# shiyao-li/NextBestPath

Hardware: AMD Instinct MI355X
Metric: exploration steps/s (+ NBP maps/s) at 256x256 (higher is better)
Workload: dtype f32

## Files before the change

include/nbp_hip.h:

```cpp
#ifndef NBP_HIP_H
#define NBP_HIP_H

#include <stddef.h>
#include <stdint.h>

#ifdef __cplusplus
extern "C" {
#endif

#define NBP_E_ARG      (-1)
#define NBP_E_WS       (-2)
#define NBP_E_SHAPE    (-3)

int nbp_abi_version(void);
int nbp_device_info(char* arch_host, int arch_len, int* cu_count_host);
int nbp_tuning_active(void);
int nbp_tuning_report(char* buf_host, int len);
int nbp_tile_kernel_symbol(int tile, char* buf_host, int len);

#define NBP_N_CONV 48

typedef struct nbp_weights nbp_weights;

size_t nbp_packed_weights_bytes(void);
// ... 57 lines not shown
int nbp_conv3x3_split_f32(const float* src0, int C0, const float* src1, int C1, int ups, int B, int H, int W,
                          const void* w_planes, const void* wamax, int N, const float* scale, const float* shift, int relu,
                          float* out, const void* amax_in_or_null, void* amax_out_or_null, int split_k, void* ws,
                          size_t ws_bytes, void* stream);
size_t nbp_conv_first_wgrad_workspace_bytes(void);
int nbp_conv_first_wgrad_f32(const float* x_nchw, int B, int H, int W, const float* dy, float* dw, void* ws, size_t ws_bytes, void* stream);
int nbp_prepack_weights_split(const void* descs_dev, int n, void* wamax_words, void* stream);
int nbp_prepack_desc_bytes(void);
int nbp_pack_conv_weight_split_prezeroed(const float* w_oihw, int N, int C, int ksize, int c_total, void* dst_planes,
                                         void* wamax_zeroed, void* stream);
int nbp_pack_conv_weight_split_dgrad_known(const float* w_oihw, int N, int C, int c_total, void* dst_planes, const void* wamax_known,
                                           void* stream);
int nbp_pack_upconv_weight_split_dgrad(const float* w_oihw, int N, int C, void* dst_planes, void* wamax_out, void* stream);
size_t nbp_upconv_split_dgrad_workspace_bytes(int B, int H, int W, int N, int C);
int nbp_upconv3x3_split_dgrad_f32(const float* dy, int N, int B, int H, int W, const void* planes, const void* wamax, int C,
                                  const float* scale, const float* shift, float* dx, const void* amax_in, void* amax_out_or_null,
                                  void* ws, size_t ws_bytes, void* stream);
size_t nbp_upconv_wgrad_split_workspace_bytes(int B, int Hs, int Ws, int C, int N);
int nbp_upconv_wgrad_split_f32(const float* x, int C, int B, int Hs, int Ws, const float* dy, int N, float* dw,
                               const void* amax_x, const void* amax_y, void* ws, size_t ws_bytes, void* stream);
int nbp_conv1x1_split_f32(const float* src, int C, long long M, const void* w_planes, const void* wamax, int N,
                          const float* scale, const float* shift, int relu, float* out, const void* amax_in, void* stream);
int nbp_pack_conv1x1_weight_split_dgrad(const float* w_nc, int N, int C, void* dst_planes, void* wamax_out, void* stream);
int nbp_pack_conv_weight_split_dgrad(const float* w_oihw, int N, int C, int c_total, void* dst_planes, void* wamax_out, void* stream);

int nbp_conv_bn_part_rows(int B, int H, int W);
int nbp_conv3x3_split_bn_f32(const float* src0, int C0, const float* src1, int C1, int ups, int B, int H, int W,
                             const void* w_planes, const void* wamax, int N, const float* scale, const float* shift, int relu,
                             float* out, const void* amax_in_or_null, void* amax_out_or_null, int split_k, void* ws,
                             size_t ws_bytes, double* bn_part, int* bn_rows, void* stream);
int nbp_upconv3x3_split_bn_f32(const float* src, int C, int B, int H, int W, const void* planes_up, const void* wamax_up, int N,
                               const float* scale, const float* shift, int relu, float* out, const void* amax_in_or_null,
                               void* amax_out_or_null, int split_k, void* ws, size_t ws_bytes, double* bn_part, int* bn_rows,
                               void* stream);
int nbp_pack_conv_weight_split_h1(const float* w_oihw, int N, int C, int ksize, const float* scale_or_null, int c_off,
                                  int c_total, void* dst_planes, void* wamax_out, void* stream);
int nbp_pack_conv_weight_split_prezeroed_h1(const float* w_oihw, int N, int C, int ksize, int c_total, void* dst_planes,
                                            void* wamax_zeroed, void* stream);
int nbp_pack_conv_weight_split_dgrad_h1(const float* w_oihw, int N, int C, int c_total, void* dst_planes, void* wamax_out, void* stream);
int nbp_pack_conv_weight_split_dgrad_known_h1(const float* w_oihw, int N, int C, int c_total, void* dst_planes, const void* wamax_known,
                                              void* stream);
int nbp_pack_upconv_weight_split_h1(const float* w_oihw, int N, int C, void* dst_planes, void* wamax_out, void* stream);
int nbp_pack_upconv_weight_split_dgrad_h1(const float* w_oihw, int N, int C, void* dst_planes, void* wamax_out, void* stream);
int nbp_pack_conv1x1_weight_split_dgrad_h1(const float* w_nc, int N, int C, void* dst_planes, void* wamax_out, void* stream);
int nbp_prepack_weights_split_h1(const void* descs_dev, int n, void* wamax_words, void* stream);
int nbp_conv3x3_split_f32_h1(const float* src0, int C0, const float* src1, int C1, int ups, int B, int H, int W,
// ... 362 lines not shown
```

nextbestpath_amd/_lib.py:

```python
from __future__ import annotations

import ctypes as C
import os
import threading

HERE = os.path.dirname(os.path.abspath(__file__))
LIB_PATH = os.path.join(HERE, "libnbp_hip.so")

_vp, _i, _ll, _f, _sz, _d = C.c_void_p, C.c_int, C.c_longlong, C.c_float, C.c_size_t, C.c_double

SIGNATURES = {
    "nbp_abi_version": (_i, []),
    "nbp_device_info": (_i, [C.c_char_p, _i, C.POINTER(_i)]),
    "nbp_tuning_active": (_i, []),
    "nbp_tuning_report": (_i, [C.c_char_p, _i]),
    "nbp_tile_kernel_symbol": (_i, [_i, C.c_char_p, _i]),
    "nbp_packed_weights_bytes": (_sz, []),
    "nbp_pack_weights": (_i, [C.POINTER(_vp), C.POINTER(_vp), C.POINTER(_vp), _vp, _sz, _vp, C.POINTER(_vp)]),
    "nbp_free_weights": (None, [_vp]),
    "nbp_forward_workspace_bytes": (_sz, [_i, _i]),
    "nbp_forward_f32": (_i, [_vp, _vp, _i, _i, _vp, _vp, _vp, _sz, _vp]),
    "nbp_forward_flops": (_d, [_i, _i]),
    "nbp_conv_igemm_f32": (_i, [_vp, _i, _vp, _i, _i, _i, _i, _i, _i, _vp, _i, _vp, _vp, _i, _vp, _i, _i, _vp,
                                _sz, _vp]),
# ... 97 lines not shown
SIGNATURES["nbp_amax_f32"] = (_i, [_vp, _ll, _vp, _vp])
SIGNATURES["nbp_pack_upconv_weight_split"] = (_i, [_vp, _i, _i, _vp, _vp, _vp])
SIGNATURES["nbp_upconv3x3_split_f32"] = (_i, [_vp, _i, _i, _i, _i, _vp, _vp, _i, _vp, _vp, _i, _vp, _vp, _vp, _i, _vp, _sz, _vp])
SIGNATURES["nbp_conv_split_workspace_bytes"] = SIGNATURES["nbp_conv_igemm_workspace_bytes"]
SIGNATURES["nbp_conv_split_planned_workspace_bytes"] = (_sz, [_i, _i, _i, _i, _i, _i, _vp])
SIGNATURES["nbp_conv_split_planned_workspace_bytes_k"] = (_sz, [_i, _i, _i, _i, _i, _i, _i, _vp])
SIGNATURES["nbp_conv3x3_split_f32"] = (_i, [_vp, _i, _vp, _i, _i, _i, _i, _i, _vp, _vp, _i, _vp, _vp, _i, _vp, _vp, _vp, _i, _vp,
                                            _sz, _vp])
SIGNATURES["nbp_pack_upconv_weight_split_dgrad"] = (_i, [_vp, _i, _i, _vp, _vp, _vp])
SIGNATURES["nbp_upconv_split_dgrad_workspace_bytes"] = (_sz, [_i, _i, _i, _i, _i])
SIGNATURES["nbp_upconv3x3_split_dgrad_f32"] = (_i, [_vp, _i, _i, _i, _i, _vp, _vp, _i, _vp, _vp, _vp, _vp, _vp, _vp, _sz, _vp])
SIGNATURES["nbp_upconv_wgrad_split_workspace_bytes"] = (_sz, [_i, _i, _i, _i, _i])
SIGNATURES["nbp_upconv_wgrad_split_f32"] = (_i, [_vp, _i, _i, _i, _i, _vp, _i, _vp, _vp, _vp, _vp, _sz, _vp])
SIGNATURES["nbp_pack_conv_weight_split_prezeroed"] = (_i, [_vp, _i, _i, _i, _i, _vp, _vp, _vp])
SIGNATURES["nbp_pack_conv_weight_split_dgrad_known"] = (_i, [_vp, _i, _i, _i, _vp, _vp, _vp])
SIGNATURES["nbp_prepack_weights_split"] = (_i, [_vp, _i, _vp, _vp])
SIGNATURES["nbp_prepack_desc_bytes"] = (_i, [])
SIGNATURES["nbp_rowscale_amax_f32"] = (_i, [_vp, _vp, _ll, _i, _vp, _vp, _vp])
SIGNATURES["nbp_conv_first_linear_f32"] = (_i, [_vp, _i, _i, _i, _vp, _vp, _vp, _vp, _vp])
SIGNATURES["nbp_conv_first_wgrad_workspace_bytes"] = (_sz, [])
SIGNATURES["nbp_conv_first_wgrad_f32"] = (_i, [_vp, _i, _i, _i, _vp, _vp, _vp, _sz, _vp])
SIGNATURES["nbp_conv1x1_split_f32"] = (_i, [_vp, _i, _ll, _vp, _vp, _i, _vp, _vp, _i, _vp, _vp, _vp])
SIGNATURES["nbp_pack_conv1x1_weight_split_dgrad"] = (_i, [_vp, _i, _i, _vp, _vp, _vp])
SIGNATURES["nbp_pack_conv_weight_split_dgrad"] = (_i, [_vp, _i, _i, _i, _vp, _vp, _vp])
SIGNATURES["nbp_conv_bn_part_rows"] = (_i, [_i, _i, _i])
SIGNATURES["nbp_conv3x3_split_bn_f32"] = (_i, [_vp, _i, _vp, _i, _i, _i, _i, _i, _vp, _vp, _i, _vp, _vp, _i, _vp, _vp, _vp, _i, _vp,
                                               _sz, _vp, C.POINTER(_i), _vp])
SIGNATURES["nbp_upconv3x3_split_bn_f32"] = (_i, [_vp, _i, _i, _i, _i, _vp, _vp, _i, _vp, _vp, _i, _vp, _vp, _vp, _i, _vp, _sz, _vp,
                                                 C.POINTER(_i), _vp])
SIGNATURES["nbp_bn_train_forward_part4_f32"] = (_i, [_vp, _ll, _i, _vp, _vp, _f, _f, _vp, _vp, _i, _vp, _vp, _vp, _vp, _vp, _i, _vp, _i, _vp, _vp])
for _n in ("nbp_pack_conv_weight_split", "nbp_pack_conv_weight_split_prezeroed", "nbp_pack_conv_weight_split_dgrad",
           "nbp_pack_conv_weight_split_dgrad_known", "nbp_pack_upconv_weight_split", "nbp_pack_upconv_weight_split_dgrad",
           "nbp_pack_conv1x1_weight_split_dgrad", "nbp_prepack_weights_split", "nbp_conv3x3_split_f32", "nbp_conv3x3_split_bn_f32",
           "nbp_upconv3x3_split_f32", "nbp_upconv3x3_split_bn_f32", "nbp_upconv3x3_split_dgrad_f32", "nbp_conv1x1_split_f32",
           "nbp_upconv_wgrad_split_f32", "nbp_conv_wgrad_split_f32"):
    SIGNATURES[_n + "_h1"] = SIGNATURES[_n]
SIGNATURES["nbp_conv_igemm_bf16"] = SIGNATURES["nbp_conv_igemm_f32"]
SIGNATURES["nbp_conv_igemm_bf16_workspace_bytes"] = SIGNATURES["nbp_conv_igemm_workspace_bytes"]
SIGNATURES["nbp_pack_conv_weight_bf16"] = SIGNATURES["nbp_pack_conv_weight"]
SIGNATURES["nbp_f32_to_bf16"] = (_i, [_vp, _ll, _vp, _vp])
SIGNATURES["nbp_bf16_to_f32"] = (_i, [_vp, _ll, _vp, _vp])
_fpp, _ipp = C.POINTER(_f), C.POINTER(_i)
SIGNATURES["nbp_scene_fill_workspace_bytes"] = (_sz, [_fpp, _ipp, _i, _ll, _d])
SIGNATURES["nbp_scene_fill_cells_f32"] = (_i, [_vp, _ll, _vp, _fpp, _ipp, _i, _d, _i, C.c_uint, _vp, _vp, _vp, _sz, _vp])
SIGNATURES["nbp_scene_gather_f32"] = (_i, [_vp, _vp, _i, _i, _vp, _ll, _vp, _vp])
SIGNATURES["nbp_scene_coverage_workspace_bytes"] = (_sz, [_fpp, _ipp, _i, _d])
# ... 82 lines not shown
            fn.argtypes = args
        _lib = handle
    return _lib


_ERR = {-1: "NBP_E_ARG (bad argument)", -2: "NBP_E_WS (workspace too small)", -3: "NBP_E_SHAPE (unsupported shape)"}


def check(rc: int, what: str) -> None:
    if rc != 0:
        msg = _ERR.get(rc, f"hipError_t {rc}" if rc > 0 else f"error {rc}")
        raise NbpHipError(f"{what} failed: {msg}")


def ptr(t) -> int:
    if t is None:
        return 0
    if not t.is_contiguous():
        raise ValueError("tensor passed to the HIP path must be contiguous")
    return t.data_ptr()


_knobs = {}
NUMERICS_KNOBS = {"NBP_CONV_PRECISION", "NBP_SPLIT_MAX_K", "NBP_SPLIT_MAX_K_SMALL", "NBP_GATE_PSI", "NBP_CONV_HEAD", "NBP_BF16_PSI",
                  "NBP_BF16_FUSE"}


def tuning_active() -> bool:
    return os.environ.get("NBP_TUNING") == "1"


def tune(name: str, default: str) -> str:
    v = default
    if tuning_active():
        e = os.environ.get(name)
        if e is not None and e != "":
            v = e
    _knobs[name] = (default, v)
    return v


def effective_knobs() -> dict:
    out = {k: v for k, (d, v) in _knobs.items() if v != d}
    if _lib is not None:
        buf = C.create_string_buffer(4096)
        if _lib.nbp_tuning_report(buf, 4096) > 0:
            for item in buf.value.decode().split(","):
# ... 18 lines not shown
```

nextbestpath_amd/csrc/nbp_forward.hip:

```cpp
#include "common.h"
#include "nbp_internal.h"
#include <stdio.h>
#include <stdlib.h>
#include <string.h>

namespace {

enum Kind { K_FIRST, K_CONV3, K_ATT_G, K_ATT_X, K_PSI, K_FINAL };
struct LayerSpec { Kind kind; int cin, cout, k; };

struct Table {
    LayerSpec L[NBP_N_CONV];
    size_t w_off[NBP_N_CONV];
    size_t s_off[NBP_N_CONV], t_off[NBP_N_CONV];
    size_t total_floats;
    size_t w3_off[NBP_N_CONV];
    size_t w3u_off[NBP_N_CONV];
    bool is_up[NBP_N_CONV];
    int up_rank[NBP_N_CONV];
    size_t total3_bytes;
    size_t wup16_off[NBP_N_CONV], total_up16_bytes;
    size_t w1_off[NBP_N_CONV];
    int gate_rank[NBP_N_CONV];
    Table() {
// ... 377 lines not shown
                    int H, int ks, int N, void* ws, size_t wsb, hipStream_t st) {
        if (ks == 1 && C1 == C0 && C0 % 64 == 0 && !ups && h->w1[li[0]] && (!o2 || h->w1[li[1]])) {
            const long long M = (long long)B * H * H;
            ConvOperandsSplit s[2];
            for (int g = 0; g < (o2 ? 2 : 1); ++g) {
                const Ops& q = g ? *o2 : o;
                s[g] = ConvOperandsSplit{q.src0, q.src1, h->w1[li[g]], q.scale, q.shift, q.out, nullptr, nullptr, h->wamax1[li[g]], nullptr,
                                         nullptr, nullptr};
                int rc = ctx.ensure(q.src0, M * C0, &s[g].amax0);
                if (!rc) rc = ctx.ensure(q.src1, M * C1, &s[g].amax1);
                if (rc) return rc;
            }
            GatePsi psi;
            for (int g = 0; g < 2; ++g) {
                const int l = li[(g && o2) ? 1 : 0] + 2;
                psi.wpsi[g] = (const float*)h->w[l]; psi.st[g] = h->scale[l]; psi.gated[g] = ctx.gated[(g && o2) ? 1 : 0];
            }
            unsigned* gslot[2] = {nullptr, nullptr};
            if (ctx.gated[0]) for (int g = 0; g < (o2 ? 2 : 1); ++g) psi.gated_amax[g] = gslot[g] = ctx.unbound();
            static const int psi_on_load = nbp_tune_int("NBP_SPLIT_PSI_ON_LOAD", 1);
            const ConvPlan pc = nbp_plan_conv_split(M, C0, (C0 + C0) / 32 * 9, 0, o2 ? 2 : 1, H, H, 3, 0);
            psi.psi_only = psi_on_load && (C0 >= 128 || psi_on_load >= 2) && ctx.gated[0] && gslot[0] && (!o2 || gslot[1]) && pc.tile != 0 &&
                           M * C0 * 4 < (1ll << 31);
            int fused = 0;
            const int rc = nbp_gate1x1_split_launch_g(s[0], o2 ? &s[1] : nullptr, C0, M, N, 1, st, ctx.gated[0] ? &psi : nullptr, &fused);
            if (fused) {
                ctx.gated_taken = true;
                for (int g = 0; g < (o2 ? 2 : 1); ++g) {
                    if (gslot[g]) ctx.bind(ctx.gated[g], gslot[g]);
                    else ctx.alias(ctx.gated[g], (g ? *o2 : o).src1);
                    if (psi.psi_only) { ctx.psi_key[g] = ctx.gated[g]; ctx.psi_x[g] = (g ? *o2 : o).src1; }
                }
            }
            return rc;
        }
        const ConvPlan p = nbp_plan_conv_split((long long)B * H * H, N, (C0 + C1) / 32 * ks * ks, 0, o2 ? 2 : 1, H, H, ks, ups);
        if (!p.tile) return PathF32::conv(ctx, h, li, o, o2, C0, C1, ups, B, H, ks, N, ws, wsb, st);
        const long long hw = (long long)B * (ups ? H / 2 : H) * (ups ? H / 2 : H);
        ConvOperandsSplit s[2];
        for (int g = 0; g < (o2 ? 2 : 1); ++g) {
            const Ops& q = g ? *o2 : o;
            s[g] = ConvOperandsSplit{q.src0, q.src1, h->w3[li[g]], q.scale, q.shift, q.out, nullptr, nullptr, h->wamax[li[g]], nullptr,
                                     h->w3u[li[g]], h->wamax_u[li[g]]};
            int rc = ctx.ensure(q.src0, hw * C0, &s[g].amax0);
            if (!rc && C1) rc = ctx.ensure(q.src1, hw * C1, &s[g].amax1);
            if (rc) return rc;
// ... 339 lines not shown
```

nextbestpath_amd/csrc/nbp_internal.h:

```cpp
#pragma once
#include "common.h"

typedef unsigned short bf16_t;

enum { NBP_TILE_AUTO = 0, NBP_TILE_128x128 = 1, NBP_TILE_256x64 = 2, NBP_TILE_256x32 = 3, NBP_TILE_128x64 = 4,
       NBP_TILE_64x128 = 5,
       NBP_TILE_HALO_128 = 6, NBP_TILE_HALO_64 = 7,
       NBP_TILE_HALO4_128 = 8, NBP_TILE_HALO4_64 = 9,
       NBP_TILE_SPLIT_HALO_64 = 10, NBP_TILE_SPLIT_UP = 11,
       NBP_TILE_HALO_UP_128 = 12, NBP_TILE_HALO_UP_64 = 13,
       NBP_TILE_RESERVED_14 = 14,
       NBP_TILE_SPLIT_HALO_R8 = 15, NBP_TILE_SPLIT_UP_R8 = 16,
       NBP_TILE_SPLIT_UP_DGRAD = 17,
       NBP_TILE_SPLIT_HALO_128 = 18,
       NBP_TILE_SPLIT_GATE = 19 };
struct TileInfo { int bm, bn; };
struct ConvPlan { int tile; int split_k; int chunks_per_split; };

struct IgemmArgs {
    const float* src0;
    const float* src1;
    int C0, C1;
    int cc0;
    int ups;
// ... 30 lines not shown

struct ConvOperandsSplit {
    const float* src0; const float* src1; const void* planes; const float* scale; const float* shift; float* out;
    const unsigned* amax0; const unsigned* amax1; const unsigned* wamax; unsigned* amax_out;
    const void* planes_up; const unsigned* wamax_up;
    const float* psi0 = nullptr;
};
ConvPlan nbp_plan_conv_split(long long M, int N, int chunks_total, int split_k, int groups, int H, int W, int ksize, int ups = 0);
int nbp_pack_upconv_weight_split_launch(const float* w_oihw, int N, int C, void* dst, unsigned* wamax_out, hipStream_t st, int one = 0);
struct ConvHead { const float* w; const float* scale; const float* shift; float* out; };
int nbp_conv_split_launch_g(const ConvOperandsSplit& o, const ConvOperandsSplit* o2, int C0, int C1, int ups, int B, int H, int W,
                            int ksize, int N, int relu, int split_k, void* ws, size_t ws_bytes, hipStream_t st,
                            float* const* pool_out = nullptr, int* pooled = nullptr, const struct ConvHead* head = nullptr,
                            int* headed = nullptr, double* bn_part = nullptr, int* bn_rows = nullptr, int one = 0);
int nbp_pack_conv_weight_split_launch(const float* w_oihw, int N, int C, int ksize, const float* scale_or_null, int c_off,
                                      int c_total, void* dst, unsigned* wamax_out, hipStream_t st, int one = 0);
int nbp_amax_launch(const float* x, long long n, unsigned* amax_inout, hipStream_t st);
int nbp_wgrad_split_launch(const float* src0, int C0, const float* src1, int C1, int ups, int B, int H, int W, const float* dy, int N,
                           int n_tiles, int splits, unsigned* amax3, const unsigned* amax0_in, const unsigned* amax1_in,
                           const unsigned* amaxy_in, float* part, hipStream_t st);
int nbp_pack_gate_weight_split_launch(const float* wg, const float* scale_g, const float* wx, const float* scale_x, int N, int C,
                                      void* dst, unsigned* wamax_out, hipStream_t st);
struct GatePsi { const float* wpsi[2]; const float* st[2]; float* gated[2]; unsigned* gated_amax[2] = {nullptr, nullptr};
                 int psi_only = 0; };
int nbp_gate1x1_split_launch_g(const ConvOperandsSplit& o, const ConvOperandsSplit* o2, int C, long long M, int N, int relu,
                               hipStream_t st, const GatePsi* psi = nullptr, int* fused = nullptr);
int nbp_conv_first_amax_launch(const float* x_nchw, int B, int H, int W, const float* w_oihw, const float* scale, const float* shift,
                               float* out_nhwc, unsigned* amax_out, int* did_amax, hipStream_t st);

struct ConvOperandsH { const bf16_t* src0; const bf16_t* src1; const bf16_t* wpk; const float* scale; const float* shift; bf16_t* out;
                       const bf16_t* wpk_up; };
ConvPlan nbp_plan_conv_bf16(long long M, int N, int chunks_total, int tile, int split_k, int groups, int H = 0, int W = 0,
                            int ksize = 0, int ups = 0);
int nbp_pack_upconv_weight_bf16_launch(const float* w_oihw, int N, int C, bf16_t* dst, hipStream_t st);
struct GatePsiH { const float* wpsi[2]; const float* st[2]; bf16_t* gated[2]; };
int nbp_conv_igemm_bf16_launch_g(const ConvOperandsH& o, const ConvOperandsH* o2, int C0, int C1, int ups, int B, int H,
                                 int W, int ksize, int N, int relu, int split_k, int tile, void* ws, size_t ws_bytes,
                                 hipStream_t st, bf16_t* const* pool_out = nullptr, int* pooled = nullptr,
                                 const struct ConvHead* head = nullptr, int* headed = nullptr, const GatePsiH* psi = nullptr,
                                 int* psi_fused = nullptr);
int nbp_conv_first_bf16_launch(const float* x_nchw, int B, int H, int W, const float* w_oihw, const float* scale,
                               const float* shift, bf16_t* out_nhwc, hipStream_t st);
int nbp_maxpool2_bf16_launch(const bf16_t* in, int B, int H, int W, int C, bf16_t* out, hipStream_t st);
int nbp_psi_gate_bf16_launch(const bf16_t* q, int F, const float* w_psi, const float* s_t2, const bf16_t* x, int C,
                             long long M, bf16_t* out, hipStream_t st);
int nbp_final_1x1_bf16_launch(const bf16_t* in, int B, int H, int W, int C, const float* w_oc, int n_out,
                              const float* scale, const float* shift, int sigmoid, float* out_nchw, hipStream_t st);
// ... 1 lines not shown
```

nextbestpath_amd/csrc/nbp_split.hip:

```cpp
#include "common.h"
#include "nbp_internal.h"
#include <cstdlib>

namespace {

typedef _Float16 f16x8 __attribute__((ext_vector_type(8)));
typedef _Float16 f16x2 __attribute__((ext_vector_type(2)));
typedef unsigned u32x4 __attribute__((ext_vector_type(4)));
typedef unsigned u32x2 __attribute__((ext_vector_type(2)));
typedef __attribute__((address_space(3))) void* lds_ptr_t;

constexpr int SPLIT_EXP = 14;
__host__ __device__ inline int amax_exponent(unsigned bits) {
    if (!bits) return SPLIT_EXP;
    int e = (int)((bits >> 23) & 255u) - 127;
    return e < -100 ? -100 : (e > 100 ? 100 : e);
}
__host__ __device__ inline float pow2f(int e) {
    union { unsigned u; float f; } v;
    v.u = (unsigned)(127 + e) << 23;
    return v.f;
}

__device__ __forceinline__ void split_pair(float x0, float x1, unsigned& h, unsigned& l) {
// ... 497 lines not shown
#ifdef NBP_DBG_TS
extern "C" int nbp_dbg_read(unsigned long long* host, unsigned* n) {
    hipDeviceSynchronize();
    hipMemcpyFromSymbol(n, HIP_SYMBOL(nbp_dbg_n), sizeof(unsigned));
    return (int)hipMemcpyFromSymbol(host, HIP_SYMBOL(nbp_dbg_ts), sizeof(unsigned long long) * 8192);
}
#endif

struct GateArgs {
    SplitOps g[2];
    int C, N, relu;
    int C1;
    long long M;
    unsigned bytes0, bytesw;
    int groups;
    const float* wpsi[2];
    const float* st[2];
    float* gated[2];
    unsigned* gated_amax[2];
    int psi_only;
};

template <bool ONE, int TN, bool PSI>
__global__ __launch_bounds__(256, 2) void gate1x1_h2_kernel(GateArgs a) {
    const SplitOps& o = a.g[blockIdx.z];
    constexpr int BN = TN * 32;
    constexpr int WST = (ONE ? 4 : 8) * BN * 16;
    constexpr int WI = WST / 1024;
    extern __shared__ __attribute__((aligned(16))) char wbuf[];
    const int tid = threadIdx.x, lane = tid & 63, wave = tid >> 6;
    const long long m = (long long)blockIdx.x * 128 + wave * 32 + (lane & 31);
    const int n0 = blockIdx.y * BN, khalf = lane >> 5;
    const unsigned ma0 = read_amax(o.amax0), ma1 = o.amax1 ? read_amax(o.amax1) : 0u;
    const int ea = amax_exponent(ma0 > ma1 ? ma0 : ma1), ew = amax_exponent(*o.wamax);
    const float sa = pow2f(SPLIT_EXP - ea);
    const int einv = ea + ew - 2 * SPLIT_EXP;
    const __amdgpu_buffer_rsrc_t rs0 = __builtin_amdgcn_make_buffer_rsrc(const_cast<float*>(o.src0), 0, a.bytes0, 0x00020000);
    const __amdgpu_buffer_rsrc_t rs1 = __builtin_amdgcn_make_buffer_rsrc(const_cast<float*>(o.src1 ? o.src1 : o.src0), 0, a.bytes0, 0x00020000);
    const __amdgpu_buffer_rsrc_t rsw = __builtin_amdgcn_make_buffer_rsrc(const_cast<void*>(o.planes), 0, a.bytesw, 0x00020000);
    constexpr unsigned OOB = 0x80000000u;
    const int stages0 = a.C >> 5, stages = stages0 + (a.C1 >> 5);
    const unsigned prow = m < a.M ? (unsigned)(m * a.C) * 4u : OOB;

    constexpr int D = 4;
    u32x4 xr[D][2][2];
    auto load_x = [&](int st, int slot) {
        const bool first = st < stages0;
// ... 7 lines not shown
            }
    };
    auto issue_w = [&](int st) {
        char* dst = wbuf + (st & 1) * WST;
#pragma unroll
        for (int k = 0; k < (WI + 3) / 4; ++k) {
            const int q = wave + 4 * k;
            if (q < WI) {
                constexpr int PER = BN / 64 > 0 ? BN / 64 : 1;
                const int r8 = BN >= 64 ? q / PER : q * 2 + (lane >> 5), nb = BN >= 64 ? q - (q / PER) * PER : 0;
                const int row = BN >= 64 ? nb * 64 + lane : (lane & 31);
                const int ks = ONE ? r8 >> 1 : r8 >> 2, r4 = ONE ? r8 & 1 : r8 & 3;
                const unsigned woff = (unsigned)((((long long)(2 * st + ks) * (ONE ? 2 : 4) + r4) * a.N + n0 + row) * 16);
                __builtin_amdgcn_raw_ptr_buffer_load_lds(rsw, (lds_ptr_t)(dst + q * 1024), 16, woff, 0, 0, 0);
            }
        }
    };

    f32x16 acc[TN];
#pragma unroll
    for (int j = 0; j < TN; ++j)
#pragma unroll
        for (int r = 0; r < 16; ++r) acc[j][r] = 0.f;

    issue_w(0);
#pragma unroll
    for (int d = 0; d < D - 1; ++d) load_x(d, d);
    asm volatile("s_waitcnt vmcnt(0)" ::: "memory");
    __syncthreads();
    for (int base = 0; base < stages; base += D) {
#pragma unroll
        for (int u = 0; u < D; ++u) {
            const int st = base + u;
            if (st + 1 < stages) issue_w(st + 1);
            load_x(st + D - 1, (u + D - 1) % D);
            const char* Bt = wbuf + (st & 1) * WST + khalf * (BN * 16) + (lane & 31) * 16;
            if (st < stages)
#pragma unroll
            for (int ks = 0; ks < 2; ++ks) {
                const f32x4 v0 = __builtin_bit_cast(f32x4, xr[u][ks][0]), v1 = __builtin_bit_cast(f32x4, xr[u][ks][1]);
                if constexpr (ONE) {
                    const u32x4 xh = u32x4{hi_pair(v0[0] * sa, v0[1] * sa), hi_pair(v0[2] * sa, v0[3] * sa), hi_pair(v1[0] * sa, v1[1] * sa),
                                           hi_pair(v1[2] * sa, v1[3] * sa)};
#pragma unroll
                    for (int j = 0; j < TN; ++j) {
                        const u32x4 wh = *reinterpret_cast<const u32x4*>(Bt + (ks * 2) * (BN * 16) + j * 512);
                        acc[j] = __builtin_amdgcn_mfma_f32_32x32x16_f16(__builtin_bit_cast(f16x8, xh), __builtin_bit_cast(f16x8, wh), acc[j], 0, 0, 0);
                    }
                    continue;
                }
                unsigned h0, l0, h1, l1, h2, l2, h3, l3;
                split_pair(v0[0] * sa, v0[1] * sa, h0, l0); split_pair(v0[2] * sa, v0[3] * sa, h1, l1);
                split_pair(v1[0] * sa, v1[1] * sa, h2, l2); split_pair(v1[2] * sa, v1[3] * sa, h3, l3);
                const u32x4 xh = u32x4{h0, h1, h2, h3}, xl = u32x4{l0, l1, l2, l3};
#pragma unroll
                for (int j = 0; j < TN; ++j) {
                    const u32x4 wh = *reinterpret_cast<const u32x4*>(Bt + ((ks * 2 + 0) * 2) * (BN * 16) + j * 512);
                    const u32x4 wl = *reinterpret_cast<const u32x4*>(Bt + ((ks * 2 + 1) * 2) * (BN * 16) + j * 512);
                    acc[j] = __builtin_amdgcn_mfma_f32_32x32x16_f16(__builtin_bit_cast(f16x8, xl), __builtin_bit_cast(f16x8, wh), acc[j], 0, 0, 0);
                    acc[j] = __builtin_amdgcn_mfma_f32_32x32x16_f16(__builtin_bit_cast(f16x8, xh), __builtin_bit_cast(f16x8, wl), acc[j], 0, 0, 0);
                    acc[j] = __builtin_amdgcn_mfma_f32_32x32x16_f16(__builtin_bit_cast(f16x8, xh), __builtin_bit_cast(f16x8, wh), acc[j], 0, 0, 0);
                }
            }
// ... 29 lines not shown
            for (int i = 0; i < 4; ++i) p4[i] = (up ? p8[4 + i] : p8[i]) + __shfl_xor(up ? p8[i] : p8[4 + i], 8);
        }
        {
            const bool up = lane & 4;
#pragma unroll
            for (int i = 0; i < 2; ++i) p2[i] = (up ? p4[2 + i] : p4[i]) + __shfl_xor(up ? p4[i] : p4[2 + i], 4);
        }
        float dot;
        {
            const bool up = lane & 2;
            dot = (up ? p2[1] : p2[0]) + __shfl_xor(up ? p2[0] : p2[1], 2);
        }
        dot += __shfl_xor(dot, 1);
        const float z = dot * a.st[blockIdx.z][0] + a.st[blockIdx.z][1];
        const float psi = 1.f / (1.f + expf(-z));
        float* psil = reinterpret_cast<float*>(wbuf) + wave * 32;
        const int r = (lane & 31) >> 1;
        if (!(lane & 1)) {
            const int pix = (r & 3) + 8 * (r >> 2) + 4 * khalf;
            psil[pix] = psi;
            if (a.psi_only && mw + pix < a.M) a.gated[blockIdx.z][mw + pix] = psi;
        }
        asm volatile("s_waitcnt lgkmcnt(0)" ::: "memory");
        const int C4 = a.C >> 2, total = 32 * C4;
        const f32x4* x4 = reinterpret_cast<const f32x4*>(o.src1) + mw * C4;
        f32x4* g4 = reinterpret_cast<f32x4*>(a.gated[blockIdx.z]) + mw * C4;
        const long long lim = (a.M - mw) * C4;
        float gmx = 0.f;
#pragma unroll 1
        for (int i0 = lane; i0 < total; i0 += 256) {
            f32x4 v[4];
#pragma unroll
            for (int u = 0; u < 4; ++u) { const int i = i0 + 64 * u; if (i < total && i < lim) v[u] = x4[i]; }
#pragma unroll
            for (int u = 0; u < 4; ++u) {
                const int i = i0 + 64 * u;
                if (i < total && i < lim) {
                    const float ps = psil[i / C4];
                    const f32x4 g = v[u] * ps;
                    if (!a.psi_only) g4[i] = g;
                    gmx = fmaxf(fmaxf(gmx, fmaxf(fabsf(g[0]), fabsf(g[1]))), fmaxf(fabsf(g[2]), fabsf(g[3])));
                }
            }
        }
        if (a.gated_amax[blockIdx.z]) wave_amax(gmx, a.gated_amax[blockIdx.z]);
    } else {
#pragma unroll
    for (int j = 0; j < TN; ++j) {
        const int n = n0 + j * 32 + (lane & 31);
        const float sc = o.scale[n], sh = o.shift[n];
#pragma unroll
        for (int r = 0; r < 16; ++r) {
            const long long mm = mw + (r & 3) + 8 * (r >> 2) + 4 * khalf;
            if (mm < a.M) {
                float v = ldexpf(acc[j][r], einv) * sc + sh;
                if (a.relu) v = fmaxf(v, 0.f);
                o.out[mm * a.N + n] = v;
            }
        }
    }
    }
}

struct WgradSplitArgs {
    const float* src0; const float* src1;
    int C0, C1, ups, H, W, Hs, Ws;
    const float* dy; int N;
    unsigned bytes0, bytes1, bytesy;
// ... 1011 lines not shown

int nbp_gate1x1_split_launch_g(const ConvOperandsSplit& o, const ConvOperandsSplit* o2, int C, long long M, int N, int relu,
                               hipStream_t st, const GatePsi* psi, int* fused) {
    const int groups = o2 ? 2 : 1;
    NBP_RETURN_IF(!o.src0 || !o.src1 || !o.planes || !o.scale || !o.shift || !o.out || !o.amax0 || !o.amax1 || !o.wamax, NBP_E_ARG);
    NBP_RETURN_IF(o2 && (!o2->src0 || !o2->src1 || !o2->planes || !o2->out || !o2->amax0 || !o2->amax1 || !o2->wamax), NBP_E_ARG);
    NBP_RETURN_IF(C < 64 || C % 64 || N < 32 || N % 32 || M < 1, NBP_E_SHAPE);
    const long long b0 = M * C * 4, bw = 2ll * C * N * 4;
    NBP_RETURN_IF(b0 >= (1ll << 31) || bw >= (1ll << 31), NBP_E_SHAPE);
    GateArgs a;
    for (int g = 0; g < 2; ++g) {
        const ConvOperandsSplit& s = (g && o2) ? *o2 : o;
        a.g[g] = SplitOps{s.src0, s.src1, s.planes, s.scale, s.shift, s.out, s.amax0, s.amax1, s.wamax, nullptr, nullptr, nullptr, {nullptr, nullptr}, nullptr};
        const int gi = g < groups ? g : 0;
        a.wpsi[g] = psi ? psi->wpsi[gi] : nullptr; a.st[g] = psi ? psi->st[gi] : nullptr; a.gated[g] = psi ? psi->gated[gi] : nullptr;
        a.gated_amax[g] = psi ? psi->gated_amax[gi] : nullptr;
    }
    a.psi_only = psi ? psi->psi_only : 0;
    a.C = C; a.C1 = C; a.N = N; a.relu = relu; a.M = M; a.bytes0 = (unsigned)b0; a.bytesw = (unsigned)bw; a.groups = groups;
    int bn = N % 128 == 0 ? 128 : (N % 64 == 0 ? 64 : 32);
    static const int allow_psi = nbp_tune_int("NBP_GATE_PSI", 1);
    const bool psi_wants_128 = allow_psi && psi && N == 128 && psi->wpsi[0] && psi->st[0] && psi->gated[0];
    if (bn == 128 && nbp_cdiv(M, 128) * (N / 128) * groups < 512 && !psi_wants_128) bn = 64;
    const bool with_psi = allow_psi && psi && bn == N && psi->wpsi[0] && psi->st[0] && psi->gated[0] &&
                          (groups == 1 || (psi->wpsi[1] && psi->st[1] && psi->gated[1]));
    if (fused) *fused = with_psi;
    dim3 grid((unsigned)nbp_cdiv(M, 128), (unsigned)(N / bn), (unsigned)groups);
    const size_t smem = 2 * (size_t)8 * bn * 16;
    {
        char nm[64];
        snprintf(nm, sizeof(nm), "gate1x1_h2_kernel<false, %d, %s>", bn / 32, with_psi ? "true" : "false");
        nbp_note_kernel_symbol(NBP_TILE_SPLIT_GATE, nm);
    }
    if (with_psi) {
        if (bn == 128) gate1x1_h2_kernel<false, 4, true><<<grid, 256, smem, st>>>(a);
        else if (bn == 64) gate1x1_h2_kernel<false, 2, true><<<grid, 256, smem, st>>>(a);
        else gate1x1_h2_kernel<false, 1, true><<<grid, 256, smem, st>>>(a);
    } else if (bn == 128) gate1x1_h2_kernel<false, 4, false><<<grid, 256, smem, st>>>(a);
    else if (bn == 64) gate1x1_h2_kernel<false, 2, false><<<grid, 256, smem, st>>>(a);
    else gate1x1_h2_kernel<false, 1, false><<<grid, 256, smem, st>>>(a);
    return nbp_launch_status();
}

int nbp_upconv_dgrad_split_launch(const float* dy, int N, int B, int H, int W, const void* planes, const unsigned* wamax,
                                  const unsigned* amax_in, int C, const float* scale, const float* shift, float* out, unsigned* amax_out,
                                  int split_k, void* ws, size_t ws_bytes, hipStream_t st, int one = 0) {
    NBP_RETURN_IF(!dy || !planes || !wamax || !amax_in || !scale || !shift || !out, NBP_E_ARG);
    NBP_RETURN_IF(B < 1 || N < 16 || N % 16 || C < 64 || C % 64, NBP_E_SHAPE);
    const int tw = split_tile_width(H, W, C, 3);
    NBP_RETURN_IF(!tw, NBP_E_SHAPE);
    SplitArgs a;
    for (int g = 0; g < 2; ++g)
        a.g[g] = SplitOps{dy, nullptr, planes, scale, shift, out, amax_in, nullptr, wamax, amax_out, nullptr, nullptr, {nullptr, nullptr}, nullptr, nullptr};
    a.C0 = N; a.C1 = 0; a.ups = 0; a.H = H; a.W = W; a.Hs = 2 * H; a.Ws = 2 * W; a.N = C; a.relu = 0; a.groups = 1;
    a.M = (long long)B * H * W;
    const long long b0 = (long long)B * 4 * H * W * N * 4, bw = 64ll * N * C;
    NBP_RETURN_IF(b0 >= (1ll << 31) || bw >= (1ll << 31), NBP_E_SHAPE);
    a.bytes0 = (unsigned)b0; a.bytes1 = (unsigned)b0; a.bytesw = (unsigned)bw;
// ... 388 lines not shown
                                         (hipStream_t)stream);
}
extern "C" int nbp_upconv3x3_split_dgrad_f32_h1(const float* dy, int N, int B, int H, int W, const void* planes, const void* wamax, int C,
                                                const float* scale, const float* shift, float* dx, const void* amax_in, void* amax_out_or_null,
                                                void* ws, size_t ws_bytes, void* stream) {
    NBP_ENTER();
    return nbp_upconv_dgrad_split_launch(dy, N, B, H, W, planes, (const unsigned*)wamax, (const unsigned*)amax_in, C, scale, shift, dx,
                                         (unsigned*)amax_out_or_null, 0, ws ? (char*)ws + 256 : nullptr, ws_bytes >= 256 ? ws_bytes - 256 : 0,
                                         (hipStream_t)stream, 1);
}

extern "C" int nbp_conv1x1_split_f32(const float* src, int C, long long M, const void* w_planes, const void* wamax, int N,
                                     const float* scale, const float* shift, int relu, float* out, const void* amax_in, void* stream) {
    NBP_ENTER();
    return nbp_conv1x1_split_launch(src, C, M, w_planes, (const unsigned*)wamax, (const unsigned*)amax_in, N, scale, shift, relu, out,
                                    (hipStream_t)stream);
}
extern "C" int nbp_conv1x1_split_f32_h1(const float* src, int C, long long M, const void* w_planes, const void* wamax, int N,
                                        const float* scale, const float* shift, int relu, float* out, const void* amax_in, void* stream) {
    NBP_ENTER();
    return nbp_conv1x1_split_launch(src, C, M, w_planes, (const unsigned*)wamax, (const unsigned*)amax_in, N, scale, shift, relu, out,
                                    (hipStream_t)stream, 1);
}
template <bool ONE>
static int pack_conv1x1_weight_split_dgrad_impl(const float* w_nc, int N, int C, void* dst_planes, void* wamax_out, void* stream) {
    NBP_RETURN_IF(!w_nc || !dst_planes || !wamax_out, NBP_E_ARG);
    NBP_RETURN_IF(N < 32 || N % 32 || C < 32 || C % 32, NBP_E_SHAPE);
    hipStream_t st = (hipStream_t)stream;
    const long long total = (long long)N * C;
    hipError_t e = hipMemsetAsync(wamax_out, 0, sizeof(unsigned), st);
    if (e != hipSuccess) return (int)e;
    amax_kernel<<<min(nbp_ew_grid(total, 256), 256), 256, 0, st>>>(w_nc, total, nullptr, C, (unsigned*)wamax_out, 1u);
    pack_conv_weight_h2_kernel<ONE><<<nbp_ew_grid(total, 256), 256, 0, st>>>(w_nc, C, N, 1, nullptr, 0, (const unsigned*)wamax_out,
                                                                            (unsigned short*)dst_planes, 1);
    return nbp_launch_status();
}
extern "C" int nbp_pack_conv1x1_weight_split_dgrad(const float* w_nc, int N, int C, void* dst_planes, void* wamax_out, void* stream) {
    NBP_ENTER();
    return pack_conv1x1_weight_split_dgrad_impl<false>(w_nc, N, C, dst_planes, wamax_out, stream);
}
extern "C" int nbp_pack_conv1x1_weight_split_dgrad_h1(const float* w_nc, int N, int C, void* dst_planes, void* wamax_out, void* stream) {
    NBP_ENTER();
    return pack_conv1x1_weight_split_dgrad_impl<true>(w_nc, N, C, dst_planes, wamax_out, stream);
}

extern "C" int nbp_pack_upconv_weight_split(const float* w_oihw, int N, int C, void* dst_planes, void* wamax_out, void* stream) {
// ... 72 lines not shown
```

Baseline: 2324.

## Add wide N=256 fused gate+psi tile and fold gated amax into x-load loop

Adds a TN=8 (BN=256) variant of the fused gate/psi 1x1 kernel, selectable via the NBP_GATE_PSI_256 knob (off by default) and always used by the new C API entry point. The gated-output amax is now computed from the running max of |x| seen during the K loop times psi, instead of in the epilogue. This lets psi-only mode skip the epilogue re-read of x entirely. It also exposes standalone pack/gate-psi C entry points, and the wide tile lowers launch bounds to one block per SIMD, which risks occupancy.

```diff
diff --git a/include/nbp_hip.h b/include/nbp_hip.h
--- a/include/nbp_hip.h
+++ b/include/nbp_hip.h
@@ -103,6 +103,14 @@
 int nbp_conv1x1_split_f32(const float* src, int C, long long M, const void* w_planes, const void* wamax, int N,
                           const float* scale, const float* shift, int relu, float* out, const void* amax_in, void* stream);
 int nbp_pack_conv1x1_weight_split_dgrad(const float* w_nc, int N, int C, void* dst_planes, void* wamax_out, void* stream);
+int nbp_pack_gate_weight_split(const float* w_g, const float* scale_g_or_null, const float* w_x, const float* scale_x_or_null,
+                               int N, int C, void* dst_planes, void* wamax_out, void* stream);
+int nbp_gate_psi_split_f32(const float* g, const float* x, int C, long long M, const void* planes, const void* wamax, int N,
+                           const float* scale, const float* shift, const float* w_psi, const float* s_t2, float* gated,
+                           void* gated_amax_or_null, const float* g_b, const float* x_b, const void* planes_b,
+                           const void* wamax_b, const float* scale_b, const float* shift_b, const float* w_psi_b,
+                           const float* s_t2_b, float* gated_b, void* gated_amax_b_or_null, int psi_only, void* ws,
+                           size_t ws_bytes, void* stream);
 int nbp_pack_conv_weight_split_dgrad(const float* w_oihw, int N, int C, int c_total, void* dst_planes, void* wamax_out, void* stream);
 
 int nbp_conv_bn_part_rows(int B, int H, int W);
diff --git a/nextbestpath_amd/_lib.py b/nextbestpath_amd/_lib.py
--- a/nextbestpath_amd/_lib.py
+++ b/nextbestpath_amd/_lib.py
@@ -143,6 +143,9 @@
 SIGNATURES["nbp_conv_first_wgrad_f32"] = (_i, [_vp, _i, _i, _i, _vp, _vp, _vp, _sz, _vp])
 SIGNATURES["nbp_conv1x1_split_f32"] = (_i, [_vp, _i, _ll, _vp, _vp, _i, _vp, _vp, _i, _vp, _vp, _vp])
 SIGNATURES["nbp_pack_conv1x1_weight_split_dgrad"] = (_i, [_vp, _i, _i, _vp, _vp, _vp])
+SIGNATURES["nbp_pack_gate_weight_split"] = (_i, [_vp, _vp, _vp, _vp, _i, _i, _vp, _vp, _vp])
+SIGNATURES["nbp_gate_psi_split_f32"] = (_i, [_vp, _vp, _i, _ll, _vp, _vp, _i, _vp, _vp, _vp, _vp, _vp, _vp,
+                                             _vp, _vp, _vp, _vp, _vp, _vp, _vp, _vp, _vp, _vp, _i, _vp, _sz, _vp])
 SIGNATURES["nbp_pack_conv_weight_split_dgrad"] = (_i, [_vp, _i, _i, _i, _vp, _vp, _vp])
 SIGNATURES["nbp_conv_bn_part_rows"] = (_i, [_i, _i, _i])
 SIGNATURES["nbp_conv3x3_split_bn_f32"] = (_i, [_vp, _i, _vp, _i, _i, _i, _i, _i, _vp, _vp, _i, _vp, _vp, _i, _vp, _vp, _vp, _i, _vp,
@@ -271,7 +274,7 @@
 
 
 _knobs = {}
-NUMERICS_KNOBS = {"NBP_CONV_PRECISION", "NBP_SPLIT_MAX_K", "NBP_SPLIT_MAX_K_SMALL", "NBP_GATE_PSI", "NBP_CONV_HEAD", "NBP_BF16_PSI",
+NUMERICS_KNOBS = {"NBP_CONV_PRECISION", "NBP_SPLIT_MAX_K", "NBP_SPLIT_MAX_K_SMALL", "NBP_GATE_PSI", "NBP_GATE_PSI_256", "NBP_CONV_HEAD", "NBP_BF16_PSI",
                   "NBP_BF16_FUSE"}
 
 
diff --git a/nextbestpath_amd/csrc/nbp_forward.hip b/nextbestpath_amd/csrc/nbp_forward.hip
--- a/nextbestpath_amd/csrc/nbp_forward.hip
+++ b/nextbestpath_amd/csrc/nbp_forward.hip
@@ -423,6 +423,8 @@
             const ConvPlan pc = nbp_plan_conv_split(M, C0, (C0 + C0) / 32 * 9, 0, o2 ? 2 : 1, H, H, 3, 0);
             psi.psi_only = psi_on_load && (C0 >= 128 || psi_on_load >= 2) && ctx.gated[0] && gslot[0] && (!o2 || gslot[1]) && pc.tile != 0 &&
                            M * C0 * 4 < (1ll << 31);
+            static const int gate256 = nbp_tune_int("NBP_GATE_PSI_256", 0);
+            psi.wide = gate256;
             int fused = 0;
             const int rc = nbp_gate1x1_split_launch_g(s[0], o2 ? &s[1] : nullptr, C0, M, N, 1, st, ctx.gated[0] ? &psi : nullptr, &fused);
             if (fused) {
diff --git a/nextbestpath_amd/csrc/nbp_internal.h b/nextbestpath_amd/csrc/nbp_internal.h
--- a/nextbestpath_amd/csrc/nbp_internal.h
+++ b/nextbestpath_amd/csrc/nbp_internal.h
@@ -76,7 +76,9 @@
 int nbp_pack_gate_weight_split_launch(const float* wg, const float* scale_g, const float* wx, const float* scale_x, int N, int C,
                                       void* dst, unsigned* wamax_out, hipStream_t st);
 struct GatePsi { const float* wpsi[2]; const float* st[2]; float* gated[2]; unsigned* gated_amax[2] = {nullptr, nullptr};
-                 int psi_only = 0; };
+                 int psi_only = 0;
+                 int must_fuse = 0;
+                 int wide = 0; };
 int nbp_gate1x1_split_launch_g(const ConvOperandsSplit& o, const ConvOperandsSplit* o2, int C, long long M, int N, int relu,
                                hipStream_t st, const GatePsi* psi = nullptr, int* fused = nullptr);
 int nbp_conv_first_amax_launch(const float* x_nchw, int B, int H, int W, const float* w_oihw, const float* scale, const float* shift,
diff --git a/nextbestpath_amd/csrc/nbp_split.hip b/nextbestpath_amd/csrc/nbp_split.hip
--- a/nextbestpath_amd/csrc/nbp_split.hip
+++ b/nextbestpath_amd/csrc/nbp_split.hip
@@ -543,7 +543,7 @@
 };
 
 template <bool ONE, int TN, bool PSI>
-__global__ __launch_bounds__(256, 2) void gate1x1_h2_kernel(GateArgs a) {
+__global__ __launch_bounds__(256, TN > 4 ? 1 : 2) void gate1x1_h2_kernel(GateArgs a) {
     const SplitOps& o = a.g[blockIdx.z];
     constexpr int BN = TN * 32;
     constexpr int WST = (ONE ? 4 : 8) * BN * 16;
@@ -597,6 +597,7 @@
     for (int j = 0; j < TN; ++j)
 #pragma unroll
         for (int r = 0; r < 16; ++r) acc[j][r] = 0.f;
+    float xmax = 0.f;
 
     issue_w(0);
 #pragma unroll
@@ -614,6 +615,11 @@
 #pragma unroll
             for (int ks = 0; ks < 2; ++ks) {
                 const f32x4 v0 = __builtin_bit_cast(f32x4, xr[u][ks][0]), v1 = __builtin_bit_cast(f32x4, xr[u][ks][1]);
+                if constexpr (PSI) {
+                    if (st >= stages0)
+                        xmax = fmaxf(fmaxf(fmaxf(xmax, fmaxf(fabsf(v0[0]), fabsf(v0[1]))), fmaxf(fabsf(v0[2]), fabsf(v0[3]))),
+                                     fmaxf(fmaxf(fabsf(v1[0]), fabsf(v1[1])), fmaxf(fabsf(v1[2]), fabsf(v1[3]))));
+                }
                 if constexpr (ONE) {
                     const u32x4 xh = u32x4{hi_pair(v0[0] * sa, v0[1] * sa), hi_pair(v0[2] * sa, v0[3] * sa), hi_pair(v1[0] * sa, v1[1] * sa),
                                            hi_pair(v1[2] * sa, v1[3] * sa)};
@@ -689,28 +695,27 @@
             if (a.psi_only && mw + pix < a.M) a.gated[blockIdx.z][mw + pix] = psi;
         }
         asm volatile("s_waitcnt lgkmcnt(0)" ::: "memory");
-        const int C4 = a.C >> 2, total = 32 * C4;
-        const f32x4* x4 = reinterpret_cast<const f32x4*>(o.src1) + mw * C4;
-        f32x4* g4 = reinterpret_cast<f32x4*>(a.gated[blockIdx.z]) + mw * C4;
-        const long long lim = (a.M - mw) * C4;
-        float gmx = 0.f;
+        if (a.gated_amax[blockIdx.z]) {
+            const float gmx = fmaxf(xmax, __shfl_xor(xmax, 32)) * psil[lane & 31];
+            wave_amax(gmx, a.gated_amax[blockIdx.z]);
+        }
+        if (!a.psi_only) {
+            const int C4 = a.C >> 2, total = 32 * C4;
+            const f32x4* x4 = reinterpret_cast<const f32x4*>(o.src1) + mw * C4;
+            f32x4* g4 = reinterpret_cast<f32x4*>(a.gated[blockIdx.z]) + mw * C4;
+            const long long lim = (a.M - mw) * C4;
 #pragma unroll 1
-        for (int i0 = lane; i0 < total; i0 += 256) {
-            f32x4 v[4];
-#pragma unroll
-            for (int u = 0; u < 4; ++u) { const int i = i0 + 64 * u; if (i < total && i < lim) v[u] = x4[i]; }
-#pragma unroll
-            for (int u = 0; u < 4; ++u) {
-                const int i = i0 + 64 * u;
-                if (i < total && i < lim) {
-                    const float ps = psil[i / C4];
-                    const f32x4 g = v[u] * ps;
-                    if (!a.psi_only) g4[i] = g;
-                    gmx = fmaxf(fmaxf(gmx, fmaxf(fabsf(g[0]), fabsf(g[1]))), fmaxf(fabsf(g[2]), fabsf(g[3])));
+            for (int i0 = lane; i0 < total; i0 += 256) {
+                f32x4 v[4];
+#pragma unroll
+                for (int u = 0; u < 4; ++u) { const int i = i0 + 64 * u; if (i < total && i < lim) v[u] = x4[i]; }
+#pragma unroll
+                for (int u = 0; u < 4; ++u) {
+                    const int i = i0 + 64 * u;
+                    if (i < total && i < lim) g4[i] = v[u] * psil[i / C4];
                 }
             }
         }
-        if (a.gated_amax[blockIdx.z]) wave_amax(gmx, a.gated_amax[blockIdx.z]);
     } else {
 #pragma unroll
     for (int j = 0; j < TN; ++j) {
@@ -1768,9 +1773,12 @@
     static const int allow_psi = nbp_tune_int("NBP_GATE_PSI", 1);
     const bool psi_wants_128 = allow_psi && psi && N == 128 && psi->wpsi[0] && psi->st[0] && psi->gated[0];
     if (bn == 128 && nbp_cdiv(M, 128) * (N / 128) * groups < 512 && !psi_wants_128) bn = 64;
+    if (allow_psi && psi && psi->wide && N == 256 && psi->wpsi[0] && psi->st[0] && psi->gated[0] &&
+        (groups == 1 || (psi->wpsi[1] && psi->st[1] && psi->gated[1]))) bn = 256;
     const bool with_psi = allow_psi && psi && bn == N && psi->wpsi[0] && psi->st[0] && psi->gated[0] &&
                           (groups == 1 || (psi->wpsi[1] && psi->st[1] && psi->gated[1]));
     if (fused) *fused = with_psi;
+    NBP_RETURN_IF(psi && psi->must_fuse && !with_psi, NBP_E_SHAPE);
     dim3 grid((unsigned)nbp_cdiv(M, 128), (unsigned)(N / bn), (unsigned)groups);
     const size_t smem = 2 * (size_t)8 * bn * 16;
     {
@@ -1779,7 +1787,8 @@
         nbp_note_kernel_symbol(NBP_TILE_SPLIT_GATE, nm);
     }
     if (with_psi) {
-        if (bn == 128) gate1x1_h2_kernel<false, 4, true><<<grid, 256, smem, st>>>(a);
+        if (bn == 256) gate1x1_h2_kernel<false, 8, true><<<grid, 256, smem, st>>>(a);
+        else if (bn == 128) gate1x1_h2_kernel<false, 4, true><<<grid, 256, smem, st>>>(a);
         else if (bn == 64) gate1x1_h2_kernel<false, 2, true><<<grid, 256, smem, st>>>(a);
         else gate1x1_h2_kernel<false, 1, true><<<grid, 256, smem, st>>>(a);
     } else if (bn == 128) gate1x1_h2_kernel<false, 4, false><<<grid, 256, smem, st>>>(a);
@@ -2214,6 +2223,49 @@
     return nbp_conv1x1_split_launch(src, C, M, w_planes, (const unsigned*)wamax, (const unsigned*)amax_in, N, scale, shift, relu, out,
                                     (hipStream_t)stream, 1);
 }
+extern "C" int nbp_pack_gate_weight_split(const float* w_g, const float* scale_g_or_null, const float* w_x, const float* scale_x_or_null,
+                                          int N, int C, void* dst_planes, void* wamax_out, void* stream) {
+    NBP_ENTER();
+    return nbp_pack_gate_weight_split_launch(w_g, scale_g_or_null, w_x, scale_x_or_null, N, C, dst_planes, (unsigned*)wamax_out,
+                                             (hipStream_t)stream);
+}
+extern "C" int nbp_gate_psi_split_f32(const float* g, const float* x, int C, long long M, const void* planes, const void* wamax, int N,
+                                      const float* scale, const float* shift, const float* w_psi, const float* s_t2, float* gated,
+                                      void* gated_amax_or_null, const float* g_b, const float* x_b, const void* planes_b,
+                                      const void* wamax_b, const float* scale_b, const float* shift_b, const float* w_psi_b,
+                                      const float* s_t2_b, float* gated_b, void* gated_amax_b_or_null, int psi_only, void* ws,
+                                      size_t ws_bytes, void* stream) {
+    NBP_ENTER();
+    NBP_RETURN_IF(!g || !x || !planes || !wamax || !scale || !shift || !w_psi || !s_t2 || !gated, NBP_E_ARG);
+    const bool two = g_b != nullptr;
+    NBP_RETURN_IF(two && (!x_b || !planes_b || !wamax_b || !scale_b || !shift_b || !w_psi_b || !s_t2_b || !gated_b), NBP_E_ARG);
+    NBP_RETURN_IF(N != 32 && N != 64 && N != 128 && N != 256, NBP_E_SHAPE);
+    NBP_RETURN_IF(C < 64 || C % 64 || M < 1 || M * C * 4 >= (1ll << 31), NBP_E_SHAPE);
+    NBP_RETURN_IF(!ws || ws_bytes < 4 * AMAX_WORDS * sizeof(unsigned), NBP_E_WS);
+    hipStream_t st = (hipStream_t)stream;
+    unsigned* slots = (unsigned*)ws;
+    hipError_t e = hipMemsetAsync(slots, 0, 4 * AMAX_WORDS * sizeof(unsigned), st);
+    if (e != hipSuccess) return (int)e;
+    ConvOperandsSplit o[2];
+    GatePsi psi;
+    for (int k = 0; k < (two ? 2 : 1); ++k) {
+        const float* gs = k ? g_b : g;
+        const float* xs = k ? x_b : x;
+        int rc = nbp_amax_launch(gs, M * C, slots + (2 * k) * AMAX_WORDS, st);
+        if (!rc) rc = nbp_amax_launch(xs, M * C, slots + (2 * k + 1) * AMAX_WORDS, st);
+        if (rc) return rc;
+        float* gd = k ? gated_b : gated;
+        o[k] = ConvOperandsSplit{gs, xs, k ? planes_b : planes, k ? scale_b : scale, k ? shift_b : shift, gd, slots + (2 * k) * AMAX_WORDS,
+                                 slots + (2 * k + 1) * AMAX_WORDS, (const unsigned*)(k ? wamax_b : wamax), nullptr, nullptr, nullptr};
+        psi.wpsi[k] = k ? w_psi_b : w_psi; psi.st[k] = k ? s_t2_b : s_t2; psi.gated[k] = gd;
+        psi.gated_amax[k] = (unsigned*)(k ? gated_amax_b_or_null : gated_amax_or_null);
+    }
+    if (!two) { psi.wpsi[1] = nullptr; psi.st[1] = nullptr; psi.gated[1] = nullptr; }
+    psi.psi_only = psi_only ? 1 : 0;
+    psi.must_fuse = 1;
+    psi.wide = 1;
+    return nbp_gate1x1_split_launch_g(o[0], two ? &o[1] : nullptr, C, M, N, 1, st, &psi, nullptr);
+}
 template <bool ONE>
 static int pack_conv1x1_weight_split_dgrad_impl(const float* w_nc, int N, int C, void* dst_planes, void* wamax_out, void* stream) {
     NBP_RETURN_IF(!w_nc || !dst_planes || !wamax_out, NBP_E_ARG);
```

New measurement: 2335, median of 6. About the same (+0.5%).
